# hmc-lair-shark-tracking/auv-sim

Measured on NVIDIA B200. Metric: edge_evals_per_s, higher is better.
Workload: dtype f32

## Files before the change

auv-sim_b200/csrc/common.cuh:

```cuda
#pragma once
#include <cuda_runtime.h>
#include <stdint.h>
#include <math.h>

#define AUV_SMS 148

namespace auv {

template <typename R, bool VERIFY> struct Ar;

template <> struct Ar<double, true> {
    typedef double R;
    static __device__ __forceinline__ R add(R a, R b) { return __dadd_rn(a, b); }
    static __device__ __forceinline__ R sub(R a, R b) { return __dsub_rn(a, b); }
    static __device__ __forceinline__ R mul(R a, R b) { return __dmul_rn(a, b); }
    static __device__ __forceinline__ R div(R a, R b) { return __ddiv_rn(a, b); }
    static __device__ __forceinline__ R sqrt(R a) { return __dsqrt_rn(a); }
    static __device__ __forceinline__ R sq2(R dx, R dy) { return __dadd_rn(__dmul_rn(dx, dx), __dmul_rn(dy, dy)); }
    static __device__ __forceinline__ void sincos(R a, R *s, R *c) { ::sincos(a, s, c); }
    static __device__ __forceinline__ R floor(R a) { return ::floor(a); }
    static __device__ __forceinline__ R fabs(R a) { return ::fabs(a); }
    static __device__ __forceinline__ R fma(R a, R b, R c) { return ::fma(a, b, c); }
    static __device__ __forceinline__ R inf() { return __longlong_as_double(0x7ff0000000000000LL); }
};
// ... 81 lines not shown
        return Draw<R>::at(key, k);
    }
    __device__ __forceinline__ bool consumed_ok(uint32_t ctr_end) const {
        return !ext || (int64_t)ctr_end <= n_ext;
    }
};

template <typename R> struct SerialStream {
    uint32_t wa, wb;
    uint32_t ctr;
    __device__ __forceinline__ void init(uint64_t key) { wa = (uint32_t)key; wb = (uint32_t)(key >> 32); ctr = 0; }
    __device__ __forceinline__ void seek(uint64_t key, uint32_t pos) {
        wa = pos * AUV_WEYL_HI + (uint32_t)key; wb = pos * AUV_WEYL_LO + (uint32_t)(key >> 32); ctr = pos;
    }
    __device__ __forceinline__ R next();
    __device__ __forceinline__ void skip(uint32_t n) { wa += n * AUV_WEYL_HI; wb += n * AUV_WEYL_LO; ctr += n; }
};
template <> __device__ __forceinline__ float SerialStream<float>::next() {
    wa += AUV_WEYL_HI; ctr++;
    return Draw<float>::from_hi(mix32a(wa));
}
template <> __device__ __forceinline__ double SerialStream<double>::next() {
    wa += AUV_WEYL_HI; wb += AUV_WEYL_LO; ctr++;
    return Draw<double>::from_words(mix32a(wa), mix32b(wb));
}

template <typename R> __device__ __forceinline__ R uniform_ab(R a, R b, R d);
template <> __device__ __forceinline__ double uniform_ab<double>(double a, double b, double d) {
    return __dadd_rn(a, __dmul_rn(__dsub_rn(b, a), d));
}
template <> __device__ __forceinline__ float uniform_ab<float>(float a, float b, float d) {
    const float w = b - a;
    return fmaf(w, d, a - w);
}

template <typename R> __device__ __forceinline__ R floordiv_pos(R t, R w) {
    typedef typename Policy<R>::A A;
    R q = sizeof(R) == 4 ? A::floor(A::div(t, w)) : A::floor(t / w);
    if (A::fma(q, w, -t) > (R)0) q -= (R)1;
    else if (A::fma(q + (R)1, w, -t) <= (R)0) q += (R)1;
    return q;
}

template <int G> struct Grp {
    int lane, gl, gbase;
    unsigned gmask;
    __device__ __forceinline__ Grp() {
        unsigned l;
        asm volatile("mov.u32 %0, %%laneid;" : "=r"(l));
        lane = (int)l;
        gl = lane & (G - 1);
        gbase = lane - gl;
        gmask = (G == 32) ? 0xffffffffu : (((1u << (G & 31)) - 1u) << gbase);
    }
    __device__ __forceinline__ void sync() const { __syncwarp(gmask); }
    __device__ __forceinline__ unsigned ballot(bool p) const {
        unsigned b = __ballot_sync(gmask, p);
        return (G == 32) ? b : ((b >> gbase) & ((1u << (G & 31)) - 1u));
    }
    template <typename T> __device__ __forceinline__ T bcast(T v, int src) const {
        return __shfl_sync(gmask, v, gbase + src);
    }
    template <typename T> __device__ __forceinline__ T up(T v, int d) const {
        return __shfl_up_sync(gmask, v, d, G);
    }
    template <typename T> __device__ __forceinline__ T xorv(T v, int m) const {
        return __shfl_xor_sync(gmask, v, m, G);
    }
};

template <int G, typename T> __device__ __forceinline__ T grp_sum(const Grp<G> &g, T v) {
#pragma unroll
    for (int m = G / 2; m > 0; m >>= 1) v += g.xorv(v, m);
    return v;
}
template <int G, typename T> __device__ __forceinline__ T grp_scan_incl(const Grp<G> &g, T v) {
#pragma unroll
    for (int d = 1; d < G; d <<= 1) {
        T o = g.up(v, d);
        if (g.gl >= d) v += o;
    }
    return v;
}
template <int G> __device__ __forceinline__ double grp_scan_serial(const Grp<G> &g, double v, double carry) {
    double acc = carry, mine = carry;
#pragma unroll 1
    for (int j = 0; j < G; j++) {
        double vj = g.bcast(v, j);
        acc = __dadd_rn(acc, vj);
        if (j == g.gl) mine = acc;
    }
    return mine;
}

extern thread_local char g_err[512];
extern long long g_launches;
int set_err(int code, const char *fmt, ...);

#define AUV_CUDA(call)                                                                         \
    do {                                                                                       \
        cudaError_t e_ = (call);                                                               \
        if (e_ != cudaSuccess)                                                                 \
            return auv::set_err(AUVRRT_ERR_CUDA, "%s:%d %s: %s", __FILE__, __LINE__, #call,    \
                                cudaGetErrorString(e_));                                       \
    } while (0)

}
```

auv-sim_b200/csrc/edge.cuh:

```cuda
#pragma once
#include "geom.cuh"

#ifndef AUV_EDGE_ONE
#define AUV_EDGE_ONE 0
#endif

namespace auv {

template <typename R> struct SteerParams {
    R d2e, dmax, neg_dmax, freq, min_dist, two_vel;
    R w_diff, o_dist, o_diff, o_vel;
};

template <int G> struct Log2 { static const int v = (G == 32) ? 5 : (G == 16) ? 4 : (G == 8) ? 3 : (G == 4) ? 2 : 1; };

template <typename R, int G, bool FLAT = true> struct GroupScratch {
    R us[FLAT ? 3 * G : 32];
    R wx[G + 1], wy[G + 1];
    unsigned char jmp[FLAT ? Log2<G>::v : 1][FLAT ? 3 * G + 4 : 4];
};

template <typename R> struct EdgeOut {
    R x, y, th, t, len;
    int nwp;
    int n_exp;
    uint32_t ctr;
    int status;
    bool safe;
    R s2; uint32_t cnt; uint64_t mask;
    R self_s2; int self_hab; bool leaf_moved;
};

__device__ __forceinline__ float sinc_small(float h) {
    float z = h * h;
    if (z > 0.25f) {
        float sn, cs;
        Ar<float, false>::sincos(h, &sn, &cs);
        return __fdividef(sn, h);
    }
    float p = fmaf(z, 2.7557319e-6f, -1.9841270e-4f);
    p = fmaf(z, p, 8.3333333e-3f);
    p = fmaf(z, p, -1.6666667e-1f);
    return fmaf(z, p, 1.0f);
}

template <typename R, int G, bool DO_COLLIDE, bool DO_COST, bool WRITE_WP, bool FLAT = false, bool ONE_CHUNK = false, bool GRIDS = false>
__device__ __forceinline__ void eval_edge(const Grp<G> &g, GroupScratch<R, G, FLAT> &sc, const EnvView<R> &env,
                                          const Stream<R> &rng, uint32_t ctr, const SteerParams<R> &sp,
                                          R px, R py, R pth, R pt, R plen, R w3, int n_hab,
                                          R *wp_out, int wp_cap, EdgeOut<R> &out) {
    typedef typename Policy<R>::A A;
    const bool VERIFY = Policy<R>::VERIFY;
    const int LOG = Log2<G>::v;

    R u0 = rng.u(ctr);
    ctr += 1;
    int n_exp = (int)A::floor(uniform_ab<R>((R)0, sp.freq, u0));
    out.n_exp = n_exp;
    out.status = 0;

    R cth = pth, cx = px, cy = py, ct = pt, clen = plen;
    R csin = 0, ccos = 0;
    if (VERIFY) A::sincos(pth, &csin, &ccos);
    int nwp = 1;
    bool hit = false, outside = false, zero_div = false, moved = false, degenerate = false, parent_clear = false, parent_many = false;
    R acc_s2 = 0; uint32_t acc_cnt = 0; uint64_t acc_mask = 0;
    R self_s2 = 0; int self_hab = -1;

    if (DO_COLLIDE) {
        if (g.gl == 0) { sc.wx[G] = px; sc.wy[G] = py; }
        const Cls pcl = env.template classify<GRIDS>(px, py);
        parent_clear = (pcl.code & 4u) != 0u;
        parent_many = (pcl.code & AUV_GRID_CIRC_MANY) != 0u;
        if (VERIFY || !AUV_EDGE_ONE || (pcl.code & AUV_GRID_SLOW)) {
            outside = !point_within_c<R>(env, pcl, px, py);
            if (!parent_clear && !parent_many) hit = point_hits_circles_c<R>(env, pcl, px, py);
        } else outside = point_unsafe_one<R>(env, pcl.code, px, py);
    }

    for (int base = 0; base < n_exp; base += G) {
        const int nact = min(G, n_exp - base);
        const bool act = g.gl < nact;
        R dist = 0, diff = 0, vt = 1;
        bool valid = false;
        if (FLAT) {
    #pragma unroll
            for (int r = 0; r < 3; r++) {
                int s = g.gl + G * r;
                sc.us[s] = (s < 3 * nact) ? rng.u(ctr + (uint32_t)s) : (R)0;
            }
            g.sync();
    #pragma unroll
            for (int r = 0; r < 3; r++) {
                int s = g.gl + G * r;
                int nx = 3 * G;
                if (s <= 3 * G - 3) {
                    R dist = uniform_ab<R>((R)0, sp.d2e, sc.us[s]);
                    R diff = uniform_ab<R>(sp.neg_dmax, sp.dmax, sc.us[s + 1]);
                    nx = s + 2 + (A::fabs(dist) > A::fabs(diff) ? 1 : 0);
                    if (nx > 3 * G) nx = 3 * G;
                }
                sc.jmp[0][s] = (unsigned char)nx;
            }
            if (g.gl == 0) {
    #pragma unroll
                for (int d = 0; d < LOG; d++) sc.jmp[d][3 * G] = (unsigned char)(3 * G);
            }
            g.sync();
    #pragma unroll
            for (int d = 1; d < LOG; d++) {
    #pragma unroll
                for (int r = 0; r < 3; r++) {
                    int s = g.gl + G * r;
                    sc.jmp[d][s] = sc.jmp[d - 1][sc.jmp[d - 1][s]];
                }
                g.sync();
            }
            int o = 0;
    #pragma unroll
            for (int d = 0; d < LOG; d++)
                if ((g.gl >> d) & 1) o = sc.jmp[d][o];
            if (act) {
                dist = uniform_ab<R>((R)0, sp.d2e, sc.us[o]);
                diff = uniform_ab<R>(sp.neg_dmax, sp.dmax, sc.us[o + 1]);
                valid = A::fabs(dist) > A::fabs(diff);
                if (valid) vt = uniform_ab<R>((R)0, sp.two_vel, sc.us[o + 2]);
            }
            int o_end = g.bcast(o + 2 + (valid ? 1 : 0), nact - 1);
            ctr += (uint32_t)o_end;

        } else {
            if (act) {
                const uint32_t p0 = ctr + 3u * (uint32_t)g.gl;
                dist = uniform_ab<R>((R)0, sp.d2e, rng.u(p0));
                diff = uniform_ab<R>(sp.neg_dmax, sp.dmax, rng.u(p0 + 1u));
                valid = A::fabs(dist) > A::fabs(diff);
                if (valid) vt = uniform_ab<R>((R)0, sp.two_vel, rng.u(p0 + 2u));
            }
            ctr += 3u * (uint32_t)nact;
        }
        R phi = 0, radius = 0, chord = 0;
        if (valid) {
            if (VERIFY) {
                R s1 = A::add(dist, diff), s2 = A::sub(dist, diff);
                R den = A::add(-s1, s2);
                R num = A::add(s1, s2);
                if (den == (R)0) zero_div = true;
                radius = A::div(num, den);
                R r2 = A::mul((R)2, radius);
                if (r2 == (R)0) zero_div = true;
                phi = A::div(num, r2);
            } else {
                if (diff == (R)0) zero_div = true;
                phi = -diff;
                chord = dist * sinc_small((float)diff * 0.5f);
            }
            if (vt == (R)0) zero_div = true;
        }
        R th;
        if (VERIFY) th = (R)grp_scan_serial<G>(g, (double)phi, (double)cth);
        else th = grp_scan_incl<G>(g, phi) + cth;
        R dx = 0, dy = 0, movement = 0, dt = 0;
        if (VERIFY) {
            R s1v, c1v;
            A::sincos(th, &s1v, &c1v);
            R s0v = g.up(s1v, 1), c0v = g.up(c1v, 1);
            if (g.gl == 0) { s0v = csin; c0v = ccos; }
            if (valid) {
                dx = A::mul(radius, A::sub(s1v, s0v));
                dy = A::mul(radius, A::add(-c1v, c0v));
                movement = A::sqrt(A::sq2(dx, dy));
                dt = A::div(movement, vt);
            }
            csin = g.bcast(s1v, G - 1); ccos = g.bcast(c1v, G - 1);
        } else {
            if (valid) {
                R sm, cm;
                A::sincos(th - (R)0.5 * phi, &sm, &cm);
                dx = chord * cm; dy = chord * sm;
                movement = chord;
                dt = A::div(movement, vt);
            }
        }
        R x, y, t, len;
        if (VERIFY) {
            x = (R)grp_scan_serial<G>(g, (double)dx, (double)cx);
            y = (R)grp_scan_serial<G>(g, (double)dy, (double)cy);
            t = (R)grp_scan_serial<G>(g, (double)dt, (double)ct);
            len = (R)grp_scan_serial<G>(g, (double)movement, (double)clen);
        } else {
            x = grp_scan_incl<G>(g, dx) + cx;
            y = grp_scan_incl<G>(g, dy) + cy;
            t = grp_scan_incl<G>(g, dt) + ct;
            len = grp_scan_incl<G>(g, movement) + clen;
        }
        const bool is_wp = valid && (movement >= sp.min_dist);
        const unsigned wpm = g.ballot(is_wp);
        const unsigned vm = g.ballot(valid);
        if (vm) moved = true;
        const int last_valid = vm ? 31 - __clz(vm) : -1;

        if (WRITE_WP) {
            if (is_wp) {
                int row = nwp - 1 + __popc(wpm & ((1u << g.gl) - 1u));
                if (row < wp_cap) {
                    R *w = wp_out + 6 * (size_t)row;
                    w[0] = x; w[1] = y; w[2] = th; w[3] = vt; w[4] = t; w[5] = len;
                }
            }
        }
        Cls cl; cl.code = AUV_GRID_ALL_AMBIG | 4u; cl.idx = -1;
        if ((DO_COLLIDE || DO_COST) && (is_wp || g.gl == last_valid)) cl = env.template classify<GRIDS>(x, y);
        if (DO_COLLIDE) {
            bool in = true, h1 = false;
            if (is_wp) {
                if (VERIFY || !AUV_EDGE_ONE) {
                    in = point_within_c<R>(env, cl, x, y);
                    if (!(cl.code & AUV_GRID_CIRC_MANY)) h1 = point_hits_circles_c<R>(env, cl, x, y);
                } else {
                    in = !point_unsafe_one<R>(env, cl.code, x, y);
                    if (__builtin_expect((cl.code & AUV_GRID_SLOW) != 0u, 0)) {
                        in = point_within_c<R>(env, cl, x, y);
                        if (!(cl.code & AUV_GRID_CIRC_MANY)) h1 = point_hits_circles_c<R>(env, cl, x, y);
                    }
                }
            }
            if (g.ballot(!in)) outside = true;
            if (g.ballot(h1)) hit = true;
            const bool circles_needed = g.ballot(is_wp && !(cl.code & 4u) && (cl.code & AUV_GRID_CIRC_MANY)) != 0u ||
                                        (base == 0 && !parent_clear && parent_many);
            if (env.K > 0 && circles_needed && !outside) {
                if (is_wp) { int slot = __popc(wpm & ((1u << g.gl) - 1u)); sc.wx[slot] = x; sc.wy[slot] = y; }
                g.sync();
                const int nw = __popc(wpm);
                bool h = false;
#pragma unroll 1
                for (int k = g.gl; k < env.K; k += G) {
                    R ccx = env.cx[k], ccy = env.cy[k];
                    R q = A::inf();
                    if (base == 0) q = A::sq2(A::sub(sc.wx[G], ccx), A::sub(sc.wy[G], ccy));
#pragma unroll 1
                    for (int j = 0; j < nw; j++) {
                        R qq = A::sq2(A::sub(sc.wx[j], ccx), A::sub(sc.wy[j], ccy));
                        q = qq < q ? qq : q;
                    }
                    if (VERIFY) h = h || (A::sqrt(q) <= env.creff[k]);
                    else h = h || (q <= env.creff2[k]);
                }
                if (g.ballot(h)) hit = true;
                g.sync();
            }
        }
        if (DO_COST) {
            const bool need = is_wp || (g.gl == last_valid);
            Contrib c; c.bin = -1; c.cell = -1; c.hab = -1;
            if (need) c = point_contrib<R>(env, x, y, t, 0xffffffffu, n_hab, cl);
            R ps2 = (R)0;
            if (c.bin >= 0 && c.cell >= 0) ps2 = A::mul(w3, env.probs[(size_t)c.bin * env.C + c.cell]);
            const bool counts = is_wp && c.bin >= 0;
            acc_s2 += grp_sum<G>(g, counts ? ps2 : (R)0);
            unsigned hm = g.ballot(counts && c.hab >= 0);
            acc_cnt += __popc(hm);
            unsigned long long mbits = (counts && c.hab >= 0) ? (1ull << c.hab) : 0ull;
            if (G == 32) {
                const unsigned lo = __reduce_or_sync(0xffffffffu, (unsigned)mbits), hi = __reduce_or_sync(0xffffffffu, (unsigned)(mbits >> 32));
                mbits = ((unsigned long long)hi << 32) | lo;
            } else {
#pragma unroll
                for (int m = G / 2; m > 0; m >>= 1) mbits |= g.xorv(mbits, m);
            }
            acc_mask |= mbits;
            if (last_valid >= 0) {
                self_s2 = g.bcast((c.bin >= 0) ? ps2 : (R)0, last_valid);
                self_hab = g.bcast((c.bin >= 0) ? c.hab : -1, last_valid);
            }
        }
        nwp += __popc(wpm);
        if (last_valid >= 0) {
            cth = g.bcast(th, last_valid); cx = g.bcast(x, last_valid); cy = g.bcast(y, last_valid);
            ct = g.bcast(t, last_valid); clen = g.bcast(len, last_valid);
        }
        g.sync();
        if (g.ballot(zero_div)) {
            if (VERIFY) out.status = 2; else degenerate = true;
            break;
        }
        if (ONE_CHUNK) break;
    }
    if (DO_COLLIDE && n_exp == 0 && env.K > 0 && !parent_clear && parent_many) {
        bool h = false;
#pragma unroll 1
        for (int k = g.gl; k < env.K; k += G) {
            R q = A::sq2(A::sub(px, env.cx[k]), A::sub(py, env.cy[k]));
            if (VERIFY) h = h || (A::sqrt(q) <= env.creff[k]);
            else h = h || (q <= env.creff2[k]);
        }
        if (g.ballot(h)) hit = true;
    }
    if (!rng.consumed_ok(ctr)) out.status = 4;
    out.x = cx; out.y = cy; out.th = cth; out.t = ct; out.len = clen;
    out.nwp = nwp; out.ctr = ctr;
    out.safe = !(hit || outside || degenerate);
    out.s2 = acc_s2; out.cnt = acc_cnt; out.mask = acc_mask;
    out.self_s2 = self_s2; out.self_hab = self_hab; out.leaf_moved = moved;
}

}
```

auv-sim_b200/csrc/plan.cu:

```cuda
#include <stdlib.h>
#include "plan_common.cuh"
#include "dubins.cuh"

#ifndef AUV_PLAN_PREFETCH
#define AUV_PLAN_PREFETCH 0
#endif

namespace auv {

#define AUV_LAUNCH_CHECK2()                                                                 \
    do {                                                                                    \
        g_launches++;                                                                       \
        cudaError_t e_ = cudaGetLastError();                                                \
        if (e_ != cudaSuccess)                                                              \
            return set_err(AUVRRT_ERR_CUDA, "%s:%d launch: %s", __FILE__, __LINE__,         \
                           cudaGetErrorString(e_));                                         \
    } while (0)

#ifndef AUV_PLAN_THREADS32
#define AUV_PLAN_THREADS32 896
#endif
#ifndef AUV_PLAN_MINB32
#define AUV_PLAN_MINB32 (896 / AUV_PLAN_THREADS32)
#endif
template <typename R, int G> struct PlanCta {
    static const int T = (sizeof(R) == 4 && G == 32) ? AUV_PLAN_THREADS32 : 128, MINB = (sizeof(R) == 4 && G == 32) ? AUV_PLAN_MINB32 : 7;
};

struct WsLayout {
    size_t slot_bytes;
    size_t rows, xy, pool, next, head, tail, count;
};

template <typename R> static WsLayout make_layout(int cap, int nb, int nchunks) {
    WsLayout L;
    size_t o = 0;
    auto take = [&](size_t bytes) { size_t r = o; o += (bytes + 127) & ~(size_t)127; return r; };
    L.rows = take(sizeof(NodeRow<R>) * (size_t)cap);
    L.xy = take(2 * sizeof(R) * (size_t)cap);
    L.pool = take(4 * 32 * (size_t)nchunks); L.next = take(4 * (size_t)nchunks);
    L.head = take(4 * (size_t)(nb + 2)); L.tail = take(4 * (size_t)(nb + 2)); L.count = take(4 * (size_t)(nb + 2));
    L.slot_bytes = o;
    return L;
}

template <typename R> struct Tree {
    NodeRow<R> *row;
    R *nx, *ny;
    int *pool, *next, *head, *tail, *count;
    __device__ __forceinline__ void bind(unsigned char *b, const WsLayout &L, int cap) {
        row = (NodeRow<R> *)(b + L.rows);
        nx = (R *)(b + L.xy); ny = nx + cap;
        pool = (int *)(b + L.pool); next = (int *)(b + L.next);
        head = (int *)(b + L.head); tail = (int *)(b + L.tail); count = (int *)(b + L.count);
    }
};

template <typename R> struct DubinsEdge {
    bool ok;
    bool safe;
    R x, y, th, t, len;
    R s2; uint32_t cnt; unsigned long long mask;
    R self_s2; int self_hab;
};
template <typename R>
__device__ __forceinline__ void dubins_edge_eval(const EnvView<R> &env, const PlanP<R> &P, R px, R py, R pth, R pt, R plen,
                                                 R sx, R sy, R sth, bool do_tests, R *rows, int room, DubinsEdge<R> &e) {
    typedef typename Policy<R>::A A;
    e.ok = false; e.safe = false; e.x = px; e.y = py; e.th = pth; e.t = pt; e.len = plen;
    e.s2 = 0; e.cnt = 0; e.mask = 0ull; e.self_s2 = 0; e.self_hab = -1;
    const DubinsPath<R> d = dubins_shortest<R>(px, py, pth, sx, sy, sth, P.rho);
    if (d.word < 0) return;
    e.ok = true;
    const R s_end = d.length < P.eta ? d.length : P.eta;
    const R step = A::div(s_end, (R)(P.W - 1));
    DubinsSampler<R> smp;
    smp.init(d, px, py, pth, P.rho);
    bool bad = false;
    if (do_tests) {
        const Cls pcl = env.classify(px, py);
        bad = point_unsafe_c<R>(env, pcl, px, py);
    }
#pragma unroll 1
    for (int k = 1; k < P.W; k++) {
        const R sk = A::mul((R)k, step);
        R x, y, th;
        smp.at(sk, x, y, th);
        const R t = A::add(pt, A::div(sk, P.vel)), len = A::add(plen, sk);
        if (do_tests) {
            const Cls cl = env.classify(x, y);
            bad = bad || point_unsafe_c<R>(env, cl, x, y);
// ... 32 lines not shown
    const int pick_mode = MODE >= 0 ? MODE : P.mode;
    extern __shared__ __align__(16) unsigned char smem[];
    const int PLAN_THREADS = PlanCta<R, G>::T;
    __shared__ GroupScratch<R, G, false> scratch[PlanCta<R, G>::T / G];
    __shared__ BestPlan<R> best_s[PlanCta<R, G>::T / G];
    __shared__ unsigned short binmeta[BS ? PlanCta<R, G>::T / G : 1][3][BS ? AUV_BINS_SMEM : 1];
    EnvView<R> env;
    {
        if (stage_mode == 0) { env.bind(blob, blob); env.bind_grid(blob, blob); }
        else if (stage_mode == 3) {
            uint64_t *bar = (uint64_t *)smem;
            const EnvHeader *gh = (const EnvHeader *)blob;
            const int plane = (gh->gnx * gh->gny * 4 + 15) & ~15;
            if (threadIdx.x == 0) mbar_init(bar, 1);
            __syncthreads();
            if (threadIdx.x == 0) {
                mbar_expect_tx(bar, (uint32_t)(total_bytes + plane));
                for (int o = 0; o < total_bytes; o += 65536) tma_bulk_g2s(smem + 16 + o, blob + o, (uint32_t)(total_bytes - o < 65536 ? total_bytes - o : 65536), bar);
                const unsigned char *gsrc = blob + gh->off_grid;
                for (int o = 0; o < plane; o += 65536) tma_bulk_g2s(smem + 16 + total_bytes + o, gsrc + o, (uint32_t)(plane - o < 65536 ? plane - o : 65536), bar);
            }
            mbar_wait(bar, 0);
            env.bind(smem + 16, smem + 16);
            env.bind_grid(blob, smem + 16);
            env.grid0s = (const unsigned *)(smem + 16 + total_bytes);
            __builtin_assume(__isShared(env.grid0s));
        } else {
            uint64_t *bar = (uint64_t *)smem;
            stage_env_tma(smem + 16, blob, stage_mode == 2 ? total_bytes : hot_bytes, bar);
            env.bind(smem + 16, stage_mode == 2 ? smem + 16 : blob);
            env.bind_grid(blob, smem + 16);
        }
        if (ONE) env.assume_hot_shared(PlanCta<R, G>::T >= 896);
    }
    Grp<G> g;
    GroupScratch<R, G, false> &sc = scratch[threadIdx.x / G];
    const int slot = blockIdx.x * (PLAN_THREADS / G) + threadIdx.x / G;
    Tree<R> T;
    T.bind(ws + (size_t)slot * L.slot_bytes, L, P.cap);
    unsigned short *s_count = binmeta[BS ? threadIdx.x / G : 0][0], *s_head = binmeta[BS ? threadIdx.x / G : 0][1],
                   *s_tail = binmeta[BS ? threadIdx.x / G : 0][2];
#define BIN_COUNT(b) (BS ? (int)s_count[b] : T.count[b])
#define BIN_HEAD(b) (BS ? (int)s_head[b] : T.head[b])
#define BIN_TAIL(b) (BS ? (int)s_tail[b] : T.tail[b])
#define SET_BIN_COUNT(b, v) do { if (BS) s_count[b] = (unsigned short)(v); else T.count[b] = (v); } while (0)
#define SET_BIN_HEAD(b, v) do { if (BS) s_head[b] = (unsigned short)(v); else T.head[b] = (v); } while (0)
#define SET_BIN_TAIL(b, v) do { if (BS) s_tail[b] = (unsigned short)(v); else T.tail[b] = (v); } while (0)

    for (;;) {
        long long q = 0;
        if (g.gl == 0) q = (long long)atomicAdd(qcounter, 1ull);
        q = g.bcast(q, 0);
        if (q >= Q) break;

        Stream<R> rng;
        rng.key = stream_key(seeds[q]); rng.ext = nullptr; rng.n_ext = 0;
        const R sx = starts[5 * q], sy = starts[5 * q + 1], sth = starts[5 * q + 2], st = starts[5 * q + 3],
                slen = starts[5 * q + 4];
        for (int b = g.gl; b < P.nb + 2; b += G) SET_BIN_COUNT(b, 0);
        if (g.gl == 0) {
            NodeRow<R> r0;
            r0.x = sx; r0.y = sy; r0.th = sth; r0.t = st; r0.len = slen;
            r0.parent = -1; r0.ctr = 0; r0.s2 = (R)0; r0.cnt = 0; r0.mask = 0ull; r0.born = 0;
            Contrib c = point_contrib<R>(env, sx, sy, st, 0xffffffffu, env.H, env.classify(sx, sy));
            r0.self_s2 = (c.bin >= 0 && c.cell >= 0) ? A::mul(P.w3, env.probs[(size_t)c.bin * env.C + c.cell]) : (R)0;
            r0.self_hab = c.bin >= 0 ? c.hab : -1;
            T.row[0] = r0;
            if (pick_mode == 1 || pick_mode == 3) { T.nx[0] = sx; T.ny[0] = sy; }
        }
        g.sync();
        if (g.gl == 0) { SET_BIN_HEAD(1, 0); SET_BIN_TAIL(1, 0); SET_BIN_COUNT(1, 1); T.pool[0] = 0; T.next[0] = -1; }
        g.sync();
        int n_nodes = 1, n_chunks = 1;
        uint32_t ctr = 0, upos_mark = 0;
        int status = AUVRRT_ST_OK;
        int n_cost_evals = 0;
        unsigned n_waypoints = 0, n_prims = 0;
        R best_total = A::inf();
        if (g.gl == 0) { BestPlan<R> b0; b0.c0 = b0.c1 = b0.c2 = b0.len = b0.t = (R)0; b0.node = -1; b0.iter = -1; best_s[threadIdx.x / G] = b0; }
        int it = 0;
        int guard = 0;
        const int guard_max = (int)min(64LL * P.I + 1024, 2147483647LL);

        while (it < P.I && guard++ < guard_max) {
            int parent;
            if (pick_mode == 3) {
                const uint32_t ctr0 = ctr;
                R smx, smy, smth;
                dubins_sample_at<R>(env, rng, ctr, smx, smy, smth);
                ctr += 4;
                int *near = (int *)sc.us;
                R bq = A::inf(), bs = A::inf();
                int bi = 0x7fffffff, nlist = 0;
                for (int i0 = 0; i0 < n_nodes; i0 += G) {
                    const int i = i0 + g.gl;
                    bool in = false;
                    if (i < n_nodes) {
                        const R qq = A::sq2(A::sub(smx, T.nx[i]), A::sub(smy, T.ny[i]));
                        if (qq < bq) {
                            if (VERIFY) { R sd = A::sqrt(qq); if (sd < bs) { bs = sd; bi = i; } }
                            else { bs = qq; bi = i; }
                            bq = qq;
                        }
                        in = VERIFY ? (A::sqrt(qq) <= P.near_r) : (qq <= P.near_r2);
                    }
                    const unsigned m = g.ballot(in);
                    if (in) {
                        const int pos = nlist + __popc(m & ((1u << g.gl) - 1u));
                        if (pos < G) near[pos] = i;
                    }
                    nlist += __popc(m);
                }
                nlist = min(nlist, G);
#pragma unroll
                for (int mm = G / 2; mm > 0; mm >>= 1) {
                    R os = g.xorv(bs, mm);
                    int oi = g.xorv(bi, mm);
                    if (os < bs || (os == bs && oi < bi)) { bs = os; bi = oi; }
                }
                const int nearest = bi;
                g.sync();
                if (T.row[nearest].t > P.max_traj) { upos_mark = ctr; continue; }
                int pn = nlist;
                for (int j = g.gl; j < nlist; j += G) if (near[j] == nearest) pn = j;
#pragma unroll
                for (int mm = G / 2; mm > 0; mm >>= 1) pn = min(pn, g.xorv(pn, mm));
                const int ncand = min(G, 1 + nlist - (pn < nlist ? 1 : 0));
                int pidx = -1;
                if (g.gl == 0) pidx = nearest;
                else if (g.gl < ncand) { const int j = g.gl - 1; pidx = near[j < pn ? j : j + 1]; }
                g.sync();
                DubinsEdge<R> de;
                de.ok = false; de.safe = false; de.x = de.y = de.th = de.t = de.len = 0; de.s2 = 0; de.cnt = 0; de.mask = 0ull;
                de.self_s2 = 0; de.self_hab = -1;
                NodeRow<R> pr;
                pr.s2 = 0; pr.self_s2 = 0; pr.cnt = 0; pr.mask = 0ull; pr.self_hab = -1; pr.t = 0;
                if (pidx >= 0) {
                    pr = T.row[pidx];
                    if (!(pr.t > P.max_traj))
                        dubins_edge_eval<R>(env, P, pr.x, pr.y, pr.th, pr.t, pr.len, smx, smy, smth, true, nullptr, 0, de);
                }
                n_waypoints += (unsigned)(P.W * __popc(g.ballot(de.ok)));
                R pre_s2 = 0, c0 = 0, c1 = 0, c2 = 0, total = A::inf();
                uint32_t pre_cnt = 0; unsigned long long pre_mask = 0;
                if (de.ok && de.safe) {
                    const int ph = pr.self_hab;
                    pre_s2 = A::add(A::add(pr.s2, pr.self_s2), de.s2);
                    pre_cnt = pr.cnt + (ph >= 0 ? 1u : 0u) + de.cnt;
                    pre_mask = pr.mask | (ph >= 0 ? (1ull << ph) : 0ull) | de.mask;
                    const uint32_t cnt = pre_cnt + (de.self_hab >= 0 ? 1u : 0u);
                    const unsigned long long mk = pre_mask | (de.self_hab >= 0 ? (1ull << de.self_hab) : 0ull);
                    c1 = A::mul(P.w2, (R)cnt);
                    c2 = A::add(pre_s2, de.self_s2);
                    if (de.t > (R)0) { c1 = A::div(c1, de.t); c2 = A::div(c2, de.t); }
                    if (env.H != 0) c0 = A::div(A::mul(P.w1, (R)__popcll(mk)), (R)env.H);
                    total = py_sum3p<R>(c0, c1, c2);
                }
                R bt = total; int bp = (de.ok && de.safe) ? pidx : 0x7fffffff;
#pragma unroll
                for (int mm = G / 2; mm > 0; mm >>= 1) {
                    R ot = g.xorv(bt, mm);
                    int op = g.xorv(bp, mm);
                    if (ot < bt || (ot == bt && op < bp)) { bt = ot; bp = op; }
                }
                const bool any_safe = bp != 0x7fffffff;
                const unsigned wm = g.ballot(any_safe && pidx == bp && de.ok && de.safe);
// ... 297 lines not shown
                w[0] = x; w[1] = y; w[2] = th; w[3] = (P.mode == 3 && e > 0) ? P.vel : (R)0; w[4] = t; w[5] = len;
            }
            n_path++;
            int room = P.path_cap - n_path; if (room < 0) room = 0;
            if (P.mode == 3) {
                R smx, smy, smth;
                dubins_sample_at<R>(env, rng, chain[(size_t)q * P.chain_cap + e], smx, smy, smth);
                DubinsEdge<R> de;
                dubins_edge_eval<R>(env, P, x, y, th, t, len, smx, smy, smth, false,
                                    g.gl == 0 ? rows + 6 * (size_t)(n_path < P.path_cap ? n_path : 0) : nullptr, room, de);
                n_path += P.W - 1;
                x = de.x; y = de.y; th = de.th; t = de.t; len = de.len;
                continue;
            }
            EdgeOut<R> o;
            eval_edge<R, G, false, false, true>(g, sc, env, rng, chain[(size_t)q * P.chain_cap + e], P.sp, x, y, th, t,
                                                len, (R)0, 0, rows + 6 * (size_t)(n_path < P.path_cap ? n_path : 0),
                                                room, o);
            n_path += o.nwp - 1;
            x = o.x; y = o.y; th = o.th; t = o.t; len = o.len;
        }
        if (d >= 0) {
            if (g.gl == 0 && n_path < P.path_cap) {
                R *w = rows + 6 * (size_t)n_path;
                w[0] = x; w[1] = y; w[2] = th; w[3] = (P.mode == 3 && d > 0) ? P.vel : (R)0; w[4] = t; w[5] = len;
            }
            n_path++;
        }
        if (g.gl == 0) n_path_out[q] = n_path;
    }
}

template <typename R, int G, bool BS, int MODE, bool ONE> static int plan_geometry(const auvrrt_env *env, int *grid, int *smem, int *stage_mode) {
    EnvBlob<R> b = env_blob<R>(env);
    int budget = sizeof(R) == 4 ? (PlanCta<R, G>::T >= 896 ? 96 * 1024 : 24 * 1024) : 110 * 1024;
    if (const char *ev = getenv("AUVRRT_PLAN_STAGE_KB")) budget = atoi(ev) * 1024;
    if (const char *ev = getenv("AUVRRT_PLAN_BUDGET_KB")) budget = atoi(ev) * 1024;
    int sm = 16, mode = 0;
    if (b.total_bytes + 16 <= budget) { sm = b.total_bytes + 16; mode = 2; }
    else if (b.hot_bytes + 16 <= budget) { sm = b.hot_bytes + 16; mode = 1; }
    if (ONE && PlanCta<R, G>::T >= 896) {
        const EnvHeader &hd = sizeof(R) == 4 ? env->h32 : env->h64;
        sm = b.total_bytes + 16 + ((hd.gnx * hd.gny * 4 + 15) & ~15); mode = 3;
    }
    AUV_CUDA(cudaFuncSetAttribute(k_plan<R, G, BS, MODE, ONE>, cudaFuncAttributeMaxDynamicSharedMemorySize, sm));
    int per_sm = 0;
    AUV_CUDA(cudaOccupancyMaxActiveBlocksPerMultiprocessor(&per_sm, k_plan<R, G, BS, MODE, ONE>, PlanCta<R, G>::T, sm));
    if (per_sm < 1) return set_err(AUVRRT_ERR_CUDA, "plan: kernel does not fit on an SM (smem %d)", sm);
    int nsm = 0, dev = 0;
    AUV_CUDA(cudaGetDevice(&dev));
    AUV_CUDA(cudaDeviceGetAttribute(&nsm, cudaDevAttrMultiProcessorCount, dev));
    *grid = nsm * per_sm; *smem = sm; *stage_mode = mode;
    return AUVRRT_OK;
}

template <typename R, int G, bool BS, int MODE, bool ONE>
static int launch_plan_gb(const auvrrt_env *env, const R *starts, const uint64_t *seeds, int64_t Q,
                         const auvrrt_plan_params_t *p, void *workspace, int64_t workspace_bytes,
                         auvrrt_plan_record_t *records, uint32_t *chain, R *path, const auvrrt_plan_trace_t *trace,
                         cudaStream_t s, int64_t *need_bytes) {
    PlanP<R> P;
    int rc = make_planp<R>(env, p, &P);
    if (rc) return rc;
    int grid, smem, mode;
    rc = plan_geometry<R, G, BS, MODE, ONE>(env, &grid, &smem, &mode);
    if (rc) return rc;
    WsLayout L = make_layout<R>(P.cap, P.nb, P.nchunks);
    const int gpc = PlanCta<R, G>::T / G;
    int64_t need = 256 + (int64_t)grid * gpc * (int64_t)L.slot_bytes;
    if (need_bytes) { *need_bytes = need; return AUVRRT_OK; }
    if (Q <= 0) return AUVRRT_OK;
    if (workspace_bytes < need) return set_err(AUVRRT_ERR_ARG, "plan: workspace too small (%lld < %lld)", (long long)workspace_bytes, (long long)need);
    if (P.trace && !trace) return set_err(AUVRRT_ERR_ARG, "plan: trace requested without trace buffers");
    int64_t blocks = (Q + gpc - 1) / gpc;
    if (blocks < grid) grid = (int)blocks;
    AUV_CUDA(cudaMemsetAsync(workspace, 0, 256, s));
    auvrrt_plan_trace_t tr;
    if (trace) tr = *trace; else { tr.parent = nullptr; tr.safe = nullptr; tr.nwp = nullptr; tr.leaf = nullptr; tr.upos = nullptr; }
    EnvBlob<R> b = env_blob<R>(env);
    k_plan<R, G, BS, MODE, ONE><<<grid, PlanCta<R, G>::T, smem, s>>>(b.blob, b.hot_bytes, b.total_bytes, mode, starts, seeds, (long long)Q, P, L,
                                                  (unsigned char *)workspace + 256, (unsigned long long *)workspace,
                                                  records, chain, path, tr);
    AUV_LAUNCH_CHECK2();
    return AUVRRT_OK;
}

template <typename R, int G>
static int launch_plan_g(const auvrrt_env *env, const R *starts, const uint64_t *seeds, int64_t Q,
                         const auvrrt_plan_params_t *p, void *workspace, int64_t workspace_bytes,
                         auvrrt_plan_record_t *records, uint32_t *chain, R *path, const auvrrt_plan_trace_t *trace,
                         cudaStream_t s, int64_t *need_bytes) {
    const double nb = ceil(p->max_traj_time / p->bin_interval);
    const bool bs = nb + 2 <= AUV_BINS_SMEM && p->iterations < 65000 && !getenv("AUVRRT_PLAN_BINS_GLOBAL");
#define AUV_PLAN_ARGS env, starts, seeds, Q, p, workspace, workspace_bytes, records, chain, path, trace, s, need_bytes
    if constexpr (sizeof(R) == 4) {
        if (p->mode == 0 && !getenv("AUVRRT_PLAN_GENERIC")) {
            const bool fits = PlanCta<R, G>::T >= 896
                                  ? (env->h32.gnx > 0 && env->h32.total_bytes + 16 + env->h32.gnx * env->h32.gny * 4 + 16 <= 180 * 1024)
                                  : env->h32.hot_bytes + 16 <= 24 * 1024;
            if (p->freq <= (double)G && bs && fits && !getenv("AUVRRT_PLAN_STAGE_KB"))
                return launch_plan_gb<R, G, true, 0, true>(AUV_PLAN_ARGS);
            return bs ? launch_plan_gb<R, G, true, 0, false>(AUV_PLAN_ARGS) : launch_plan_gb<R, G, false, 0, false>(AUV_PLAN_ARGS);
        }
    }
    return bs ? launch_plan_gb<R, G, true, -1, false>(AUV_PLAN_ARGS) : launch_plan_gb<R, G, false, -1, false>(AUV_PLAN_ARGS);
#undef AUV_PLAN_ARGS
}

template <typename R>
int launch_plan(const auvrrt_env *env, const R *starts, const uint64_t *seeds, int64_t Q,
                const auvrrt_plan_params_t *p, void *workspace, int64_t workspace_bytes,
                auvrrt_plan_record_t *records, uint32_t *chain, R *path, const auvrrt_plan_trace_t *trace,
                cudaStream_t s) {
    int G = p->group ? p->group : ((Q >= 32768 && !(path && p->path_cap > 0) && p->mode != 3) ? 1 : 32);
    if (G == 1 && p->mode == 3) return set_err(AUVRRT_ERR_UNSUPPORTED, "plan: mode 3 evaluates one candidate parent per lane; group must be 32, 16 or 8");
    if (G == 1) {
        if (path && p->path_cap > 0) return set_err(AUVRRT_ERR_UNSUPPORTED, "plan: group 1 (thread per tree) writes no paths; use auvrrt_materialize");
        return launch_plan_tpt<R>(env, starts, seeds, Q, p, workspace, workspace_bytes, records, chain, trace, s, nullptr);
    }
    if (G == 32) return launch_plan_g<R, 32>(env, starts, seeds, Q, p, workspace, workspace_bytes, records, chain, path, trace, s, nullptr);
    if (G == 16) return launch_plan_g<R, 16>(env, starts, seeds, Q, p, workspace, workspace_bytes, records, chain, path, trace, s, nullptr);
    if (G == 8) return launch_plan_g<R, 8>(env, starts, seeds, Q, p, workspace, workspace_bytes, records, chain, path, trace, s, nullptr);
    return set_err(AUVRRT_ERR_ARG, "plan: group must be 32, 16, 8 or 1");
}
template <typename R>
int64_t plan_workspace_bytes(const auvrrt_env *env, const auvrrt_plan_params_t *p, int64_t Q) {
    int64_t need = -1;
    int G = p->group ? p->group : ((Q >= 32768 && p->mode != 3) ? 1 : 32), rc;
    if (G == 1) rc = launch_plan_tpt<R>(env, nullptr, nullptr, Q, p, nullptr, 0, nullptr, nullptr, nullptr, 0, &need);
    else if (G == 32) rc = launch_plan_g<R, 32>(env, nullptr, nullptr, 0, p, nullptr, 0, nullptr, nullptr, nullptr, nullptr, 0, &need);
    else if (G == 16) rc = launch_plan_g<R, 16>(env, nullptr, nullptr, 0, p, nullptr, 0, nullptr, nullptr, nullptr, nullptr, 0, &need);
    else if (G == 8) rc = launch_plan_g<R, 8>(env, nullptr, nullptr, 0, p, nullptr, 0, nullptr, nullptr, nullptr, nullptr, 0, &need);
    else { set_err(AUVRRT_ERR_ARG, "plan: group must be 32, 16, 8 or 1"); return -1; }
    return rc ? -1 : need;
}
template int launch_plan<float>(const auvrrt_env *, const float *, const uint64_t *, int64_t, const auvrrt_plan_params_t *,
                                void *, int64_t, auvrrt_plan_record_t *, uint32_t *, float *, const auvrrt_plan_trace_t *, cudaStream_t);
template int launch_plan<double>(const auvrrt_env *, const double *, const uint64_t *, int64_t, const auvrrt_plan_params_t *,
                                 void *, int64_t, auvrrt_plan_record_t *, uint32_t *, double *, const auvrrt_plan_trace_t *, cudaStream_t);
template int64_t plan_workspace_bytes<float>(const auvrrt_env *, const auvrrt_plan_params_t *, int64_t);
template int64_t plan_workspace_bytes<double>(const auvrrt_env *, const auvrrt_plan_params_t *, int64_t);

template <typename R>
int launch_materialize(const auvrrt_env *env, const R *starts, const uint64_t *seeds, const uint32_t *chain,
                       const int32_t *depth, int64_t Q, const auvrrt_plan_params_t *p, R *path, int32_t *n_path,
                       cudaStream_t s) {
    if (Q <= 0) return AUVRRT_OK;
    PlanP<R> P;
    int rc = make_planp<R>(env, p, &P);
    if (rc) return rc;
    int64_t blocks = (Q + 3) / 4;
    if (blocks > AUV_SMS * 8) blocks = AUV_SMS * 8;
    k_materialize<R, 32><<<(unsigned)blocks, 128, 0, s>>>(env_blob<R>(env).blob, starts, seeds, chain, depth, (long long)Q, P, path, n_path);
    AUV_LAUNCH_CHECK2();
    return AUVRRT_OK;
}
template int launch_materialize<float>(const auvrrt_env *, const float *, const uint64_t *, const uint32_t *, const int32_t *,
                                       int64_t, const auvrrt_plan_params_t *, float *, int32_t *, cudaStream_t);
template int launch_materialize<double>(const auvrrt_env *, const double *, const uint64_t *, const uint32_t *, const int32_t *,
                                        int64_t, const auvrrt_plan_params_t *, double *, int32_t *, cudaStream_t);

}
```

Measured before the change: 1.130 billion.

## Pack two speculative RRT edge expansions into one warp via segmented scans

Adds a paired-iteration path to the fp32 single-chunk plan kernel. It speculatively samples the next parent and, when both edges' expansion counts fit in 32 lanes, evaluates both edges in one warp using segmented scans, sums and ballots. The aim is to fill the lanes that sit idle when an edge has few primitives. The cost is extra sampling work, more complex control flow, and speculation that is discarded when the second edge conflicts with the first (same bin, empty or reset bin).

```diff
diff --git a/auv-sim_b200/csrc/common.cuh b/auv-sim_b200/csrc/common.cuh
--- a/auv-sim_b200/csrc/common.cuh
+++ b/auv-sim_b200/csrc/common.cuh
@@ -187,6 +187,23 @@
     }
     return v;
 }
+template <int G, typename T> __device__ __forceinline__ T seg_scan_incl(const Grp<G> &g, T v, int j) {
+#pragma unroll
+    for (int d = 1; d < G; d <<= 1) {
+        T o = g.up(v, d);
+        if (j >= d) v += o;
+    }
+    return v;
+}
+template <int G, typename T> __device__ __forceinline__ T seg_sum(const Grp<G> &g, T v, int s, int j, int w) {
+#pragma unroll
+    for (int m = G / 2; m > 0; m >>= 1) {
+        const int p = j ^ m;
+        const T o = g.bcast(v, s + (p < w ? p : j));
+        v += p < w ? o : (T)0;
+    }
+    return g.bcast(v, s);
+}
 template <int G> __device__ __forceinline__ double grp_scan_serial(const Grp<G> &g, double v, double carry) {
     double acc = carry, mine = carry;
 #pragma unroll 1
diff --git a/auv-sim_b200/csrc/edge.cuh b/auv-sim_b200/csrc/edge.cuh
--- a/auv-sim_b200/csrc/edge.cuh
+++ b/auv-sim_b200/csrc/edge.cuh
@@ -44,14 +44,19 @@
     return fmaf(z, p, 1.0f);
 }
 
-template <typename R, int G, bool DO_COLLIDE, bool DO_COST, bool WRITE_WP, bool FLAT = false, bool ONE_CHUNK = false, bool GRIDS = false>
+template <typename R, int G, bool DO_COLLIDE, bool DO_COST, bool WRITE_WP, bool FLAT = false, bool ONE_CHUNK = false, bool GRIDS = false,
+          bool SEG = false>
 __device__ __forceinline__ void eval_edge(const Grp<G> &g, GroupScratch<R, G, FLAT> &sc, const EnvView<R> &env,
                                           const Stream<R> &rng, uint32_t ctr, const SteerParams<R> &sp,
                                           R px, R py, R pth, R pt, R plen, R w3, int n_hab,
-                                          R *wp_out, int wp_cap, EdgeOut<R> &out) {
+                                          R *wp_out, int wp_cap, EdgeOut<R> &out, int seg_s = 0, int seg_w = G) {
     typedef typename Policy<R>::A A;
     const bool VERIFY = Policy<R>::VERIFY;
     const int LOG = Log2<G>::v;
+    static_assert(!SEG || (G == 32 && sizeof(R) == 4 && ONE_CHUNK && !FLAT && !WRITE_WP), "segmented edges: fp32 single-chunk warps");
+    const int j = SEG ? g.gl - seg_s : g.gl;
+    const unsigned smask = SEG ? (seg_w >= 32 ? 0xffffffffu : (1u << seg_w) - 1u) << seg_s : 0xffffffffu;
+    auto sballot = [&](bool p) -> unsigned { const unsigned b = g.ballot(p); return SEG ? (b & smask) >> seg_s : b; };
 
     R u0 = rng.u(ctr);
     ctr += 1;
@@ -68,7 +73,6 @@
     R self_s2 = 0; int self_hab = -1;
 
     if (DO_COLLIDE) {
-        if (g.gl == 0) { sc.wx[G] = px; sc.wy[G] = py; }
         const Cls pcl = env.template classify<GRIDS>(px, py);
         parent_clear = (pcl.code & 4u) != 0u;
         parent_many = (pcl.code & AUV_GRID_CIRC_MANY) != 0u;
@@ -78,9 +82,9 @@
         } else outside = point_unsafe_one<R>(env, pcl.code, px, py);
     }
 
-    for (int base = 0; base < n_exp; base += G) {
+    for (int base = 0; SEG ? base == 0 : base < n_exp; base += G) {
         const int nact = min(G, n_exp - base);
-        const bool act = g.gl < nact;
+        const bool act = j < nact;
         R dist = 0, diff = 0, vt = 1;
         bool valid = false;
         if (FLAT) {
@@ -131,7 +135,7 @@
 
         } else {
             if (act) {
-                const uint32_t p0 = ctr + 3u * (uint32_t)g.gl;
+                const uint32_t p0 = ctr + 3u * (uint32_t)j;
                 dist = uniform_ab<R>((R)0, sp.d2e, rng.u(p0));
                 diff = uniform_ab<R>(sp.neg_dmax, sp.dmax, rng.u(p0 + 1u));
                 valid = A::fabs(dist) > A::fabs(diff);
@@ -159,6 +163,7 @@
         }
         R th;
         if (VERIFY) th = (R)grp_scan_serial<G>(g, (double)phi, (double)cth);
+        else if (SEG) th = seg_scan_incl(g, phi, j) + cth;
         else th = grp_scan_incl<G>(g, phi) + cth;
         R dx = 0, dy = 0, movement = 0, dt = 0;
         if (VERIFY) {
@@ -188,6 +193,11 @@
             y = (R)grp_scan_serial<G>(g, (double)dy, (double)cy);
             t = (R)grp_scan_serial<G>(g, (double)dt, (double)ct);
             len = (R)grp_scan_serial<G>(g, (double)movement, (double)clen);
+        } else if (SEG) {
+            x = seg_scan_incl(g, dx, j) + cx;
+            y = seg_scan_incl(g, dy, j) + cy;
+            t = seg_scan_incl(g, dt, j) + ct;
+            len = seg_scan_incl(g, movement, j) + clen;
         } else {
             x = grp_scan_incl<G>(g, dx) + cx;
             y = grp_scan_incl<G>(g, dy) + cy;
@@ -195,8 +205,8 @@
             len = grp_scan_incl<G>(g, movement) + clen;
         }
         const bool is_wp = valid && (movement >= sp.min_dist);
-        const unsigned wpm = g.ballot(is_wp);
-        const unsigned vm = g.ballot(valid);
+        const unsigned wpm = sballot(is_wp);
+        const unsigned vm = sballot(valid);
         if (vm) moved = true;
         const int last_valid = vm ? 31 - __clz(vm) : -1;
 
@@ -210,7 +220,7 @@
             }
         }
         Cls cl; cl.code = AUV_GRID_ALL_AMBIG | 4u; cl.idx = -1;
-        if ((DO_COLLIDE || DO_COST) && (is_wp || g.gl == last_valid)) cl = env.template classify<GRIDS>(x, y);
+        if ((DO_COLLIDE || DO_COST) && (is_wp || j == last_valid)) cl = env.template classify<GRIDS>(x, y);
         if (DO_COLLIDE) {
             bool in = true, h1 = false;
             if (is_wp) {
@@ -225,14 +235,19 @@
                     }
                 }
             }
-            if (g.ballot(!in)) outside = true;
-            if (g.ballot(h1)) hit = true;
-            const bool circles_needed = g.ballot(is_wp && !(cl.code & 4u) && (cl.code & AUV_GRID_CIRC_MANY)) != 0u ||
+            if (sballot(!in)) outside = true;
+            if (sballot(h1)) hit = true;
+            const bool circles_needed = sballot(is_wp && !(cl.code & 4u) && (cl.code & AUV_GRID_CIRC_MANY)) != 0u ||
                                         (base == 0 && !parent_clear && parent_many);
-            if (env.K > 0 && circles_needed && !outside) {
-                if (is_wp) { int slot = __popc(wpm & ((1u << g.gl) - 1u)); sc.wx[slot] = x; sc.wy[slot] = y; }
+            unsigned todo = g.ballot(env.K > 0 && circles_needed && !outside && j == 0);
+            while (todo) {
+                const int l = __ffs(todo) - 1;
+                todo &= todo - 1u;
+                const bool mine = !SEG || seg_s == l;
+                if (mine && is_wp) { int slot = __popc(wpm & ((1u << j) - 1u)); sc.wx[slot] = x; sc.wy[slot] = y; }
+                if (g.gl == l) { sc.wx[G] = px; sc.wy[G] = py; }
                 g.sync();
-                const int nw = __popc(wpm);
+                const int nw = g.bcast(__popc(wpm), l);
                 bool h = false;
 #pragma unroll 1
                 for (int k = g.gl; k < env.K; k += G) {
@@ -247,22 +262,29 @@
                     if (VERIFY) h = h || (A::sqrt(q) <= env.creff[k]);
                     else h = h || (q <= env.creff2[k]);
                 }
-                if (g.ballot(h)) hit = true;
+                if (g.ballot(h) && mine) hit = true;
                 g.sync();
             }
         }
         if (DO_COST) {
-            const bool need = is_wp || (g.gl == last_valid);
+            const bool need = is_wp || (j == last_valid);
             Contrib c; c.bin = -1; c.cell = -1; c.hab = -1;
             if (need) c = point_contrib<R>(env, x, y, t, 0xffffffffu, n_hab, cl);
             R ps2 = (R)0;
             if (c.bin >= 0 && c.cell >= 0) ps2 = A::mul(w3, env.probs[(size_t)c.bin * env.C + c.cell]);
             const bool counts = is_wp && c.bin >= 0;
-            acc_s2 += grp_sum<G>(g, counts ? ps2 : (R)0);
-            unsigned hm = g.ballot(counts && c.hab >= 0);
+            if (SEG) acc_s2 += seg_sum(g, counts ? ps2 : (R)0, seg_s, j, seg_w);
+            else acc_s2 += grp_sum<G>(g, counts ? ps2 : (R)0);
+            unsigned hm = sballot(counts && c.hab >= 0);
             acc_cnt += __popc(hm);
             unsigned long long mbits = (counts && c.hab >= 0) ? (1ull << c.hab) : 0ull;
-            if (G == 32) {
+            if (SEG) {
+                const bool a = seg_s == 0;
+                const unsigned lo = (unsigned)mbits, hi = (unsigned)(mbits >> 32);
+                const unsigned loa = __reduce_or_sync(0xffffffffu, a ? lo : 0u), hia = __reduce_or_sync(0xffffffffu, a ? hi : 0u);
+                const unsigned lob = __reduce_or_sync(0xffffffffu, a ? 0u : lo), hib = __reduce_or_sync(0xffffffffu, a ? 0u : hi);
+                mbits = a ? ((unsigned long long)hia << 32) | loa : ((unsigned long long)hib << 32) | lob;
+            } else if (G == 32) {
                 const unsigned lo = __reduce_or_sync(0xffffffffu, (unsigned)mbits), hi = __reduce_or_sync(0xffffffffu, (unsigned)(mbits >> 32));
                 mbits = ((unsigned long long)hi << 32) | lo;
             } else {
@@ -270,24 +292,33 @@
                 for (int m = G / 2; m > 0; m >>= 1) mbits |= g.xorv(mbits, m);
             }
             acc_mask |= mbits;
-            if (last_valid >= 0) {
+            if (SEG) {
+                const int lv = seg_s + (last_valid >= 0 ? last_valid : 0);
+                const R s2v = g.bcast((c.bin >= 0) ? ps2 : (R)0, lv);
+                const int hv = g.bcast((c.bin >= 0) ? c.hab : -1, lv);
+                if (last_valid >= 0) { self_s2 = s2v; self_hab = hv; }
+            } else if (last_valid >= 0) {
                 self_s2 = g.bcast((c.bin >= 0) ? ps2 : (R)0, last_valid);
                 self_hab = g.bcast((c.bin >= 0) ? c.hab : -1, last_valid);
             }
         }
         nwp += __popc(wpm);
-        if (last_valid >= 0) {
+        if (SEG) {
+            const int lv = seg_s + (last_valid >= 0 ? last_valid : 0);
+            const R a = g.bcast(th, lv), b = g.bcast(x, lv), c = g.bcast(y, lv), d = g.bcast(t, lv), e = g.bcast(len, lv);
+            if (last_valid >= 0) { cth = a; cx = b; cy = c; ct = d; clen = e; }
+        } else if (last_valid >= 0) {
             cth = g.bcast(th, last_valid); cx = g.bcast(x, last_valid); cy = g.bcast(y, last_valid);
             ct = g.bcast(t, last_valid); clen = g.bcast(len, last_valid);
         }
         g.sync();
-        if (g.ballot(zero_div)) {
+        if (sballot(zero_div)) {
             if (VERIFY) out.status = 2; else degenerate = true;
             break;
         }
         if (ONE_CHUNK) break;
     }
-    if (DO_COLLIDE && n_exp == 0 && env.K > 0 && !parent_clear && parent_many) {
+    if (!SEG && DO_COLLIDE && n_exp == 0 && env.K > 0 && !parent_clear && parent_many) {
         bool h = false;
 #pragma unroll 1
         for (int k = g.gl; k < env.K; k += G) {
diff --git a/auv-sim_b200/csrc/plan.cu b/auv-sim_b200/csrc/plan.cu
--- a/auv-sim_b200/csrc/plan.cu
+++ b/auv-sim_b200/csrc/plan.cu
@@ -1,3 +1,4 @@
+#include <stdio.h>
 #include <stdlib.h>
 #include "plan_common.cuh"
 #include "dubins.cuh"
@@ -6,7 +7,15 @@
 #define AUV_PLAN_PREFETCH 0
 #endif
 
+#ifndef AUV_PLAN_PAIR
+#define AUV_PLAN_PAIR 1
+#endif
+
 namespace auv {
+
+#ifdef AUV_PLAN_PAIR_STATS
+__device__ unsigned long long g_pair_stats[5];
+#endif
 
 #define AUV_LAUNCH_CHECK2()                                                                 \
     do {                                                                                    \
@@ -205,6 +214,180 @@
         int guard = 0;
         const int guard_max = (int)min(64LL * P.I + 1024, 2147483647LL);
 
+#if AUV_PLAN_PAIR
+        if constexpr (sizeof(R) == 4 && G == 32 && BS && MODE == 0 && ONE) {
+            auto n_expand = [&](uint32_t c) { return (int)A::floor(uniform_ab<R>((R)0, P.sp.freq, rng.u(c))); };
+            bool held = false;
+            int h_par = 0; uint32_t h_ctr = 0;
+#ifdef AUV_PLAN_PAIR_STATS
+            unsigned st_pass = 0, st_packed = 0, st_spec = 0, st_drop = 0;
+#endif
+            while (it < P.I) {
+                int s_par = -1, s_bin = 0, nA = 0;
+                uint32_t s_ctr = 0, pc = ctr;
+                for (int k = held ? 1 : 0; k < 2; k++) {
+                    if (k == 1) {
+                        nA = n_expand(h_ctr);
+                        if (it + 1 >= P.I) break;
+                        pc = h_ctr + 1u + 3u * (uint32_t)nA;
+                    }
+                    int ran_bin = 0, bincnt = 0;
+                    bool kerr = false;
+                    for (;;) {
+                        R u = rng.u(pc + (uint32_t)g.gl);
+                        int rb = (int)uniform_ab<R>((R)1, (R)(P.nb + 1), u);
+                        bool ke = rb > P.nb || rb < 1;
+                        int cn = ke ? 0 : (int)s_count[rb];
+                        unsigned m = g.ballot(ke || cn > 0);
+                        if (m) {
+                            int f = __ffs(m) - 1;
+                            ran_bin = g.bcast(rb, f); bincnt = g.bcast(cn, f); kerr = g.bcast(ke ? 1 : 0, f) != 0;
+                            pc += (uint32_t)f + 1u;
+                            break;
+                        }
+                        pc += G;
+                    }
+                    int par = -1;
+                    if (!kerr) {
+                        R u = rng.u(pc);
+                        pc += 1;
+                        int idx = (int)uniform_ab<R>((R)0, (R)bincnt, u);
+                        if (idx < bincnt) {
+                            int ch = s_head[ran_bin];
+#pragma unroll 1
+                            for (int hop = idx >> 5; hop > 0; hop--) ch = T.next[ch];
+                            par = T.pool[ch * 32 + (idx & 31)];
+                        }
+                    }
+                    if (k == 0) {
+                        if (par < 0) { ctr = pc; status = AUVRRT_ST_KEY_ERROR; break; }
+                        h_par = par; h_ctr = pc; held = true;
+                    } else if (par >= 0) { s_par = par; s_bin = ran_bin; s_ctr = pc; }
+                }
+                if (status != AUVRRT_ST_OK) break;
+                g.sync();
+                const int nB = s_par >= 0 ? n_expand(s_ctr) : 0;
+                const int wA = max(nA, 1);
+                const bool packed = s_par >= 0 && wA + max(nB, 1) <= 32;
+                const bool inB = packed && g.gl >= wA;
+                const int parent = inB ? s_par : h_par;
+                const uint32_t ctr0 = inB ? s_ctr : h_ctr;
+                const float4 p0 = *(const float4 *)&T.row[parent];
+                const R plen = T.row[parent].len;
+                EdgeOut<R> o;
+                eval_edge<R, G, true, true, false, false, true, true, true>(g, sc, env, rng, ctr0, P.sp, p0.x, p0.y, p0.z, p0.w, plen, P.w3,
+                                                                          env.H, nullptr, 0, o, inB ? wA : 0, inB ? 32 - wA : (packed ? wA : 32));
+                const unsigned safe_bits = g.ballot(o.safe);
+#ifdef AUV_PLAN_PAIR_STATS
+                st_pass++; st_spec += s_par >= 0 ? 1u : 0u;
+#endif
+                for (int k = 0; k < 2; k++) {
+                    const int L = k ? wA : 0;
+                    const bool own = g.gl == L;
+                    const bool safe = ((safe_bits >> L) & 1u) != 0u;
+                    const R ot = g.bcast(o.t, L);
+                    n_waypoints += (unsigned)g.bcast(o.nwp, L); n_prims += k ? nB : nA;
+                    if (P.trace && own) {
+                        size_t r = (size_t)q * P.I + it;
+                        tr.parent[r] = parent; tr.safe[r] = o.safe ? 1 : 0; tr.nwp[r] = o.nwp; tr.upos[r] = upos_mark;
+                        R *lf = (R *)tr.leaf + 5 * r;
+                        lf[0] = o.x; lf[1] = o.y; lf[2] = o.th; lf[3] = o.t; lf[4] = o.len;
+                    }
+                    ctr = k ? s_ctr + 1u + 3u * (uint32_t)nB : h_ctr + 1u + 3u * (uint32_t)nA;
+                    bool conflict = false;
+                    if (safe) {
+                        const int id = n_nodes++;
+                        R pre_s2 = 0, self_s2n = 0;
+                        uint32_t pre_cnt = 0; unsigned long long pre_mask = 0; int self_habn = -1;
+                        if (own) {
+                            const NodeRow<R> pr = T.row[parent];
+                            const int ph = pr.self_hab;
+                            pre_s2 = A::add(A::add(pr.s2, pr.self_s2), o.s2);
+                            pre_cnt = pr.cnt + (ph >= 0 ? 1u : 0u) + o.cnt;
+                            pre_mask = pr.mask | (ph >= 0 ? (1ull << ph) : 0ull) | o.mask;
+                            self_s2n = o.leaf_moved ? o.self_s2 : pr.self_s2;
+                            self_habn = o.leaf_moved ? o.self_hab : ph;
+                            NodeRow<R> nr;
+                            nr.x = o.x; nr.y = o.y; nr.th = o.th; nr.t = o.t; nr.len = o.len; nr.parent = parent; nr.ctr = ctr0;
+                            nr.s2 = pre_s2; nr.cnt = pre_cnt; nr.mask = pre_mask; nr.self_s2 = self_s2n; nr.self_hab = self_habn;
+                            nr.born = it;
+                            T.row[id] = nr;
+                        }
+                        R fd = floordiv_pos<R>(ot, P.bin_interval);
+                        R fidx = fd + (R)1;
+                        R curr_bin = A::mul(fidx, P.bin_interval);
+                        int bidx = -1; bool reset = false;
+                        if (curr_bin > P.max_traj) {
+                            if (fidx >= (R)1 && fidx <= (R)P.nb) { bidx = (int)fidx; reset = true; }
+                        } else {
+                            if (fidx >= (R)1 && fidx <= (R)P.nb) bidx = (int)fidx; else status = AUVRRT_ST_KEY_ERROR;
+                        }
+                        if (bidx >= 0) {
+                            const int c_old = g.bcast(g.gl == 0 ? (int)s_count[bidx] : 0, 0);
+                            conflict = bidx == s_bin || c_old == 0 || reset;
+                            const bool reuse_head = reset && c_old > 0;
+                            const int c = reset ? 0 : c_old;
+                            const bool alloc = ((c & 31) == 0) && !reuse_head;
+                            const int nc = n_chunks;
+                            if (alloc) n_chunks++;
+                            if (g.gl == 0) {
+                                int tl = reuse_head ? s_head[bidx] : s_tail[bidx];
+                                if (alloc) {
+                                    T.next[nc] = -1;
+                                    if (c == 0) s_head[bidx] = (unsigned short)nc; else T.next[tl] = nc;
+                                    tl = nc;
+                                }
+                                s_tail[bidx] = (unsigned short)tl;
+                                T.pool[tl * 32 + (c & 31)] = id;
+                                s_count[bidx] = (unsigned short)(c + 1);
+                            }
+                        }
+                        if (status != AUVRRT_ST_OK) break;
+                        if (ot >= P.horizon) {
+                            R c0 = 0, c1 = 0, c2 = 0, total = 0;
+                            if (own) {
+                                uint32_t cnt = pre_cnt + (self_habn >= 0 ? 1u : 0u);
+                                unsigned long long mk = pre_mask | (self_habn >= 0 ? (1ull << self_habn) : 0ull);
+                                c1 = A::mul(P.w2, (R)cnt);
+                                c2 = A::add(pre_s2, self_s2n);
+                                if (o.t > (R)0) { c1 = A::div(c1, o.t); c2 = A::div(c2, o.t); }
+                                if (env.H != 0) c0 = A::div(A::mul(P.w1, (R)__popcll(mk)), (R)env.H);
+                                total = py_sum3p<R>(c0, c1, c2);
+                            }
+                            total = g.bcast(total, L);
+                            n_cost_evals++;
+                            if (total < best_total) {
+                                best_total = total;
+                                if (own) {
+                                    BestPlan<R> b; b.c0 = c0; b.c1 = c1; b.c2 = c2; b.len = o.len; b.t = o.t; b.node = id; b.iter = it;
+                                    best_s[threadIdx.x / G] = b;
+                                }
+                            }
+                        }
+                        g.sync();
+                    }
+                    it++;
+                    upos_mark = ctr;
+                    if (k == 1) break;
+                    const bool keep = s_par >= 0 && !conflict;
+#ifdef AUV_PLAN_PAIR_STATS
+                    st_drop += s_par >= 0 && conflict ? 1u : 0u; st_packed += keep && packed ? 2u : 0u;
+#endif
+                    held = keep && !packed;
+                    if (held) { h_par = s_par; h_ctr = s_ctr; }
+                    if (!(keep && packed)) break;
+                }
+                if (status != AUVRRT_ST_OK) break;
+            }
+#ifdef AUV_PLAN_PAIR_STATS
+            if (g.gl == 0) {
+                atomicAdd(&g_pair_stats[0], (unsigned long long)st_pass); atomicAdd(&g_pair_stats[1], (unsigned long long)it);
+                atomicAdd(&g_pair_stats[2], (unsigned long long)st_packed); atomicAdd(&g_pair_stats[3], (unsigned long long)st_spec);
+                atomicAdd(&g_pair_stats[4], (unsigned long long)st_drop);
+            }
+#endif
+        } else
+#endif
         while (it < P.I && guard++ < guard_max) {
             int parent;
             if (pick_mode == 3) {
@@ -668,6 +851,17 @@
                                                   (unsigned char *)workspace + 256, (unsigned long long *)workspace,
                                                   records, chain, path, tr);
     AUV_LAUNCH_CHECK2();
+#ifdef AUV_PLAN_PAIR_STATS
+    if (sizeof(R) == 4 && G == 32 && BS && MODE == 0 && ONE) {
+        unsigned long long st[5];
+        static const unsigned long long zero[5] = {0, 0, 0, 0, 0};
+        AUV_CUDA(cudaStreamSynchronize(s));
+        AUV_CUDA(cudaMemcpyFromSymbol(st, g_pair_stats, sizeof st));
+        AUV_CUDA(cudaMemcpyToSymbol(g_pair_stats, zero, sizeof zero));
+        fprintf(stderr, "plan_pair_stats {\"passes\": %llu, \"iterations\": %llu, \"packed\": %llu, \"seconds\": %llu, \"discarded\": %llu}\n",
+                st[0], st[1], st[2], st[3], st[4]);
+    }
+#endif
     return AUVRRT_OK;
 }
 
```

Measured after the change: 1.187 billion, median of 6. 5.0% higher.
